# 0x002A/MuCHSALSA

Hardware: AMD Instinct MI355X
Metric: overlap-pairs/s (higher is better)
Workload: dtype int32+f64; 1 GPU; 100k synthetic Nanopore x10 kb, 500k unitig anchors, 10x coverage (BASELINE.json configs[2]); rows=5059558, reads=100000, anchors=499992, edges=981460, edgematches_rank0=25532466, orders_rank0=1029308, parallelism=one job on one GPU, edges_proven_clean_rank0=5372

## Files before the change

### include/msgpu.h

```cpp
#ifndef MSGPU_H
#define MSGPU_H

#include <stddef.h>
#include <stdint.h>

#ifdef __cplusplus
extern "C" {
#endif

#define MSGPU_VERSION 1

#define MSGPU_OK 0
#define MSGPU_E_IO (-1)
#define MSGPU_E_FORMAT (-2)
#define MSGPU_E_NUMBER (-3)
#define MSGPU_E_NOMEM (-4)
#define MSGPU_E_ARG (-5)
#define MSGPU_E_HIP (-6)
#define MSGPU_E_STATE (-7)
#define MSGPU_E_IDS (-8)
#define MSGPU_E_NODEVICE (-9)
#define MSGPU_E_LAYOUT (-10)
#define MSGPU_E_TIMEOUT (-11)

// ... 147 lines not shown


int msgpu_load_rows(msgpu_ctx *ctx, const msgpu_row *rows, size_t n_rows);
int msgpu_load_rows_packed(msgpu_ctx *ctx, const msgpu_packed_rows *packed);
int msgpu_load_rows_device(msgpu_ctx *ctx, const void *d_rows, size_t n_rows);


int msgpu_calculate_edges(msgpu_ctx *ctx);


int msgpu_chaining_and_overlaps(msgpu_ctx *ctx);


int msgpu_get_counts(msgpu_ctx *ctx, msgpu_counts *out);
int msgpu_get_timings(msgpu_ctx *ctx, msgpu_timings *out);
int msgpu_set_stage_events(msgpu_ctx *ctx, int on);

int msgpu_copy_tables(msgpu_ctx *ctx, msgpu_edge *edges, msgpu_edgematch *ems, msgpu_order *orders, uint32_t *ids);
int msgpu_copy_tables_device(msgpu_ctx *ctx, void *d_edges, void *d_ems, void *d_orders, void *d_ids);
int msgpu_copy_reads(msgpu_ctx *ctx, int32_t *read_len, uint32_t *read_first_line);

int msgpu_merge_gathered(msgpu_ctx *ctx, const void *d_gathered, uint32_t world, const uint64_t *counts,
                         uint64_t slab_bytes, uint64_t off_edges, uint64_t off_orders, uint64_t off_ids, void *d_edges,
                         void *d_orders, void *d_ids);

int msgpu_merge_gathered_ex(msgpu_ctx *ctx, const void *d_gathered, uint32_t world, const uint64_t *counts,
                            uint64_t slab_bytes, uint64_t off_edges, uint64_t off_orders, uint64_t off_ids,
                            const uint32_t *id_base, void *d_edges, void *d_orders, void *d_ids, void *hip_stream);

uint64_t msgpu_wire_edges_bytes(uint64_t n_edges);
// ... 336 lines not shown
```

### muchsalsa_amd/_lib.py

```python
import ctypes as C
import os

import numpy as np

_HERE = os.path.dirname(os.path.abspath(__file__))
LIB_PATH = os.environ.get("MSGPU_LIB") or os.path.join(_HERE, "libmsgpu.so")

ROW_DTYPE = np.dtype([("anchor_id", "<u4"), ("read_id", "<u4"), ("read_len", "<i4"), ("i_lo", "<i4"),
                      ("i_hi", "<i4"), ("n_lo", "<i4"), ("n_hi", "<i4"), ("score", "<u4"), ("line", "<u4"),
                      ("flags", "<u4")])
EDGE_DTYPE = np.dtype([("v1", "<u4"), ("v2", "<u4"), ("em_off", "<u8"), ("order_off", "<u8"), ("em_cnt", "<u4"),
                       ("order_cnt", "<u2"), ("shadow", "u1"), ("pad", "u1")])
EM_DTYPE = np.dtype([("ov_lo", "<i4"), ("ov_hi", "<i4"), ("score", "<f8"), ("anchor_id", "<u4"), ("line", "<u4"),
                     ("flags", "<u4"), ("edge_idx", "<u4")])
ORDER_DTYPE = np.dtype([("edge_idx", "<u4"), ("flags", "<u4"), ("left_offset", "<f8"), ("right_offset", "<f8"),
                        ("score", "<u8"), ("ids_off", "<u8"), ("ids_cnt", "<u4"), ("start", "<u4"), ("end", "<u4"),
                        ("base", "<u4"), ("pad", "<u4", (2,))])
COPY_DTYPE = np.dtype([("src_off", "<u8"), ("dst_off", "<u8"), ("len", "<u4"), ("flags", "<u4")])
assert (ROW_DTYPE.itemsize, EDGE_DTYPE.itemsize, EM_DTYPE.itemsize, ORDER_DTYPE.itemsize) == (40, 32, 32, 64)
assert COPY_DTYPE.itemsize == 24
COPY_ILLUMINA, COPY_REVCOMP = 1, 2
PATH_READ_DTYPE = np.dtype([("read_id", "<u4"), ("direction", "<u4"), ("nanopore_length", "<u8")])
PATH_ORDER_DTYPE = np.dtype([("score", "<u8"), ("base_read", "<u4"), ("ids_off", "<u4"), ("ids_cnt", "<u4"),
                             ("pad", "<u4")])
# ... 111 lines not shown
    ("msgpu_parse_paf", C.c_int, [C.c_char_p, C.POINTER(Params), C.POINTER(C.c_void_p)]),
    ("msgpu_paf_free", None, [C.c_void_p]),
    ("msgpu_paf_rows", C.c_void_p, [C.c_void_p, C.POINTER(C.c_size_t)]),
    ("msgpu_paf_line_count", C.c_size_t, [C.c_void_p]),
    ("msgpu_paf_read_count", C.c_uint32, [C.c_void_p]),
    ("msgpu_paf_anchor_count", C.c_uint32, [C.c_void_p]),
    ("msgpu_paf_read_name", C.c_char_p, [C.c_void_p, C.c_uint32]),
    ("msgpu_paf_anchor_name", C.c_char_p, [C.c_void_p, C.c_uint32]),
    ("msgpu_paf_register_sequences", C.c_int, [C.c_void_p, C.c_int, C.c_void_p, C.c_void_p, C.POINTER(C.c_uint32)]),
    ("msgpu_load_rows", C.c_int, [C.c_void_p, C.c_void_p, C.c_size_t]),
    ("msgpu_load_rows_device", C.c_int, [C.c_void_p, C.c_void_p, C.c_size_t]),
    ("msgpu_calculate_edges", C.c_int, [C.c_void_p]),
    ("msgpu_chaining_and_overlaps", C.c_int, [C.c_void_p]),
    ("msgpu_get_counts", C.c_int, [C.c_void_p, C.POINTER(Counts)]),
    ("msgpu_get_timings", C.c_int, [C.c_void_p, C.POINTER(Timings)]),
    ("msgpu_set_stage_events", C.c_int, [C.c_void_p, C.c_int]),
    ("msgpu_copy_tables", C.c_int, [C.c_void_p, C.c_void_p, C.c_void_p, C.c_void_p, C.c_void_p]),
    ("msgpu_copy_tables_device", C.c_int, [C.c_void_p, C.c_void_p, C.c_void_p, C.c_void_p, C.c_void_p]),
    ("msgpu_copy_reads", C.c_int, [C.c_void_p, C.c_void_p, C.c_void_p]),
    ("msgpu_merge_gathered", C.c_int, [C.c_void_p, C.c_void_p, C.c_uint32, C.c_void_p, C.c_uint64, C.c_uint64,
                                       C.c_uint64, C.c_uint64, C.c_void_p, C.c_void_p, C.c_void_p]),
    ("msgpu_merge_gathered_ex", C.c_int, [C.c_void_p, C.c_void_p, C.c_uint32, C.c_void_p, C.c_uint64, C.c_uint64,
                                          C.c_uint64, C.c_uint64, C.c_void_p, C.c_void_p, C.c_void_p, C.c_void_p,
                                          C.c_void_p]),
    ("msgpu_wire_edges_bytes", C.c_uint64, [C.c_uint64]),
    ("msgpu_wire_orders_bytes", C.c_uint64, [C.c_uint64]),
    ("msgpu_wire_ids_bytes", C.c_uint64, [C.c_uint64, C.c_uint32]),
    ("msgpu_pack_wire", C.c_int, [C.c_void_p, C.c_void_p, C.c_void_p, C.c_void_p, C.c_uint32]),
    ("msgpu_merge_wire", C.c_int, [C.c_void_p, C.c_void_p, C.c_uint32, C.c_void_p, C.c_uint64, C.c_uint64, C.c_uint64,
                                   C.c_uint64, C.c_uint32, C.c_void_p, C.c_void_p, C.c_void_p, C.c_void_p, C.c_void_p]),
# ... 167 lines not shown
```

### muchsalsa_amd/csrc/msgpu_api.hip

```cpp
#include <hip/hip_runtime.h>

#include <chrono>
#include <cmath>
#include <cstdarg>
#include <cstdio>
#include <cstdlib>
#include <cstring>
#include <condition_variable>
#include <deque>
#include <mutex>
#include <new>
#include <thread>
#include <vector>
#include <algorithm>
#include <sys/mman.h>
#include <unistd.h>

#include "asm_internal.h"
#include "host_pool.h"
#include "msgpu.h"
#include "msgpu_internal.h"

using namespace msgpu;

// ... 207 lines not shown
  uint32_t V = 0, A = 0;
  const msgpu_row *d_rows = nullptr;

  uint64_t n_edges = 0, n_ems = 0, n_orders = 0, n_ids = 0, n_visit = 0, total_bound = 0;
  uint32_t n_list[4] = {0, 0, 0, 0};

  DevBuf rows_in, rows_pk, cnt_read, read_off, cursor, bkt_key, bkt_dead, by_read, read_cnt, alive_rank,
      anchor_cnt, anchor_off, anchor_first, anchor_off_gen, bkt2_idx, bkt2_line, by_anchor, read_len, read_first, scalars,
      scan_tmp, vis16, spos2, visits, bin_cursor, bin_start;
  DevBuf bound, cand_off, cand_j, cand_t, scr_v2, scr_start, n_cand, n_edge, lists, edges, edge_cand;
  DevBuf big_key, big_t, big_r2s, big_pfx, pair_tab, chain_chunks, big_off, cand_sums, bucket_visits;
  hipStream_t side_stream = nullptr, side_stream2 = nullptr;
  hipEvent_t  ev_side[2]  = {nullptr, nullptr}, ev_side2 = nullptr;
  uint64_t    n_big_edges = 0, n_big_ems = 0;
  bool   fast_path = true;
  bool   sub_wave  = true;
  bool   use_fork  = true;
  bool   use_prologue = true;
  bool   chain_serial = false;
  uint32_t n_cls[4] = {0, 0, 0, 0};
  uint64_t n_edges_fast = 0;
  DevBuf ems, order_scr, ids_scr, edge_norders, edge_nids, orders, ids, big_list, cls_list, big_elems,
      big_paths;
  DevBuf g_deg, g_off, g_adj, g_cand, g_sane, g_out;
  DevBuf sel_idx, sel_cnt, sel_off, sel_ems;

  DevBuf      alt_edges, alt_ems, alt_orders, alt_ids;
  hipStream_t copy_stream = nullptr;
  hipEvent_t  ev_done[2] = {nullptr, nullptr}, ev_copied[2] = {nullptr, nullptr}, ev_wall[2] = {nullptr, nullptr};
  struct HostBuf {
    void  *p   = nullptr;
    size_t cap = 0;
  } h_edges, h_ems, h_orders, h_ids, h_read_len, h_read_first, h_sel_off, h_sel_ems, h_wire[2];
  hipEvent_t ev_part[2][3] = {{nullptr, nullptr, nullptr}, {nullptr, nullptr, nullptr}};
  std::mutex              gate_m;
  std::condition_variable gate_cv;
// ... 470 lines not shown
    return MSGPU_E_HIP;
  }
  c->stream = c->own_stream;
  if (hipHostMalloc(reinterpret_cast<void **>(&c->h_scalars), (SC_COUNT + 1) * sizeof(uint64_t),
                    hipHostMallocMapped | hipHostMallocCoherent) != hipSuccess) {
    c->h_scalars = nullptr;
    msgpu_destroy(c);
    return MSGPU_E_NOMEM;
  }
  memset(c->h_scalars, 0, (SC_COUNT + 1) * sizeof(uint64_t));
  if (hipHostGetDevicePointer(reinterpret_cast<void **>(&c->h_scalars_dev), c->h_scalars, 0) != hipSuccess) c->h_scalars_dev = nullptr;
  c->readback_mapped = c->h_scalars_dev && !getenv("MSGPU_SYNC_READBACK");
  {
    const char *nf = getenv("MSGPU_NO_FASTPATH");
    c->fast_path   = !(nf && nf[0] == '1');
    const char *ns = getenv("MSGPU_NO_SUBWAVE");
    c->sub_wave    = !(ns && ns[0] == '1');
    const char *nw = getenv("MSGPU_NO_WIRE_COPY");
    c->wire_copy   = !(nw && nw[0] == '1');
    const char *nbin = getenv("MSGPU_NO_BIN");
    c->use_bin       = !(nbin && nbin[0] == '1');
    c->use_prologue = !getenv("MSGPU_NO_PROLOGUE");
    c->use_fork     = !getenv("MSGPU_NO_FORK");
    c->chain_serial = getenv("MSGPU_CHAIN_SERIAL") != nullptr;
  }
  for (auto &ev : c->ev)
    if (hipEventCreate(&ev) != hipSuccess) {
      msgpu_destroy(c);
      return MSGPU_E_HIP;
    }
// ... 392 lines not shown
  a.n_edges      = E;
  a.cand_j       = c->cand_j.as<uint32_t>();
  a.cand_t       = c->cand_t.as<uint32_t>();
  a.read_off     = c->read_off.as<uint32_t>();
  a.read_cnt     = c->read_cnt.as<uint32_t>();
  a.read_len     = c->read_len.as<int32_t>();
  a.by_read      = c->by_read.as<IRow>();
  a.by_anchor    = c->by_anchor.as<IRow>();
  a.ems          = c->ems.as<msgpu_edgematch>();
  a.order_scr    = c->order_scr.as<msgpu_order>();
  a.ids_scr      = c->ids_scr.as<uint32_t>();
  a.edge_norders = c->edge_norders.as<uint32_t>();
  a.edge_nids    = c->edge_nids.as<uint32_t>();
  a.err          = scalar<uint32_t>(c, SC_ERR);
  if (!c->pair_tab.p) {
    ENSURE(c, pair_tab, 4 * PAIR_TAB_STRIDE * sizeof(uint32_t) + PAIR_TAB_STRIDE * sizeof(uint2) + 3 * PAIR_TAB_STRIDE * 8);
    launch_fill_pair_tab(st, c->pair_tab.as<uint32_t>());
  }
  a.pair_tab     = c->pair_tab.as<uint32_t>();
  a.pair_tab64   = c->pair_tab.as<uint32_t>() + 4 * PAIR_TAB_STRIDE;
  a.pair_tab_sub = c->pair_tab.as<uint32_t>() + 4 * PAIR_TAB_STRIDE + 2 * PAIR_TAB_STRIDE;
  if (!c->chain_zeroed)
    HIPCHK(c, hipMemsetAsync(c->chain_chunks.p, 0, chunk_words(E) * 8, st));
  c->chain_zeroed = false;
  a.chunk_sums   = c->chain_chunks.as<unsigned long long>();
  a.fast_path    = c->fast_path ? 1 : 0;
  a.fast_margin  = static_cast<long long>(std::min<uint64_t>(c->p.wiggle_room, uint64_t(1) << 40)) - 3;
  a.wiggle       = static_cast<double>(c->p.wiggle_room);
  a.ratio_pct    = c->p.ratio_pct;
  a.alt_frac     = c->p.alt_frac;
  a.out_edge_base = static_cast<uint32_t>(c->base_edges);

  const uint32_t n_big = static_cast<uint32_t>(c->n_big_edges);
  if (n_big) {
    ENSURE(c, big_elems, (c->n_big_ems ? c->n_big_ems : 1) * big_elem_bytes());
    ENSURE(c, big_paths, (c->n_big_ems ? c->n_big_ems : 1) * 2 * big_path_bytes());
  }
  if (n_big) HIPCHK(c, hipEventRecord(c->ev_side[0], st));
  auto launch_big = [&]() -> int {
    if (!n_big) return MSGPU_OK;
    HIPCHK(c, hipStreamWaitEvent(c->side_stream, c->ev_side[0], 0));
// ... 90 lines not shown
int msgpu_get_counts(msgpu_ctx *c, msgpu_counts *out) {
  if (!c || !out) return MSGPU_E_ARG;
  memset(out, 0, sizeof(*out));
  out->n_rows_in       = c->n_rows;
  out->n_rows_alive    = c->n_alive;
  out->n_reads         = c->V;
  out->n_anchors       = c->A;
  out->n_edges         = c->state >= ST_EDGES ? c->n_edges : 0;
  out->n_ems           = c->state >= ST_EDGES ? c->n_ems : 0;
  out->n_orders        = c->state >= ST_CHAINED ? c->n_orders : 0;
  out->n_ids           = c->state >= ST_CHAINED ? c->n_ids : 0;
  out->n_pairs_scanned = c->state >= ST_EDGES ? c->n_visit : 0;
  out->n_edges_fastpath = c->state >= ST_CHAINED ? c->n_edges_fast : 0;
  out->n_lost_publications = c->lost_publications;
  out->index_path          = c->index_path;
  return MSGPU_OK;
}

int msgpu_get_timings(msgpu_ctx *c, msgpu_timings *out) {
  if (!c || !out) return MSGPU_E_ARG;
  memset(out, 0, sizeof(*out));
  HIPCHK(c, hipStreamSynchronize(c->stream));
  if (c->have_index_t) HIPCHK(c, hipEventElapsedTime(&out->index_ms, c->ev[0], c->ev[1]));
  if (c->have_cand_t) HIPCHK(c, hipEventElapsedTime(&out->candidates_ms, c->ev[2], c->ev[3]));
  if (c->have_chain_t) {
    if (c->have_stage_t) {
      HIPCHK(c, hipEventElapsedTime(&out->chain_ms, c->ev[4], c->ev[7]));
      HIPCHK(c, hipEventElapsedTime(&out->compact_ms, c->ev[7], c->ev[8]));
    }
    double   sum = 0;
// ... 721 lines not shown
```

### muchsalsa_amd/csrc/msgpu_internal.h

```cpp
#ifndef MSGPU_INTERNAL_H
#define MSGPU_INTERNAL_H

#include <hip/hip_runtime.h>
#include <stdint.h>

#include "msgpu.h"

namespace msgpu {

struct IRow {
  int32_t  n_lo, n_hi, i_lo, i_hi;
  uint32_t score, line, other, pf;
};
static_assert(sizeof(IRow) == 32, "IRow must be 32 bytes");
constexpr uint32_t PF_POS_MASK = 0x3fffffffu;
constexpr uint32_t PF_DIR      = 1u << 30;
constexpr uint32_t PF_PRIM     = 1u << 31;

enum { SC_MAXIDS = 0 , SC_ERR = 1, SC_TOTAL_A = 2, SC_TOTAL_B = 3, SC_TOTAL_C = 4, SC_NLISTS = 5 ,
       SC_NBIG = 7, SC_NALIVE = 8, SC_IXFLAGS = 9, SC_BIGSTATS = 10 , SC_BIGCUR = 12 ,
       SC_CLS = 14 ,
       SC_HEADS = 16 , SC_DONE = 17 ,
       SC_OWN = 18 , SC_COUNT = 19 };
static_assert(SC_COUNT <= 64, "one wavefront publishes the whole scalar block (publish_to_host)");
// ... 210 lines not shown
void launch_rank_anchor(hipStream_t st, const uint32_t *anchor_off, uint64_t n_rows, const uint32_t *d_n_alive,
                        const uint32_t *bkt_idx, const uint32_t *bkt_line, const msgpu_row *rows,
                        const uint32_t *alive_rank, IRow *by_anchor, const uint32_t *flags, const uint32_t *read_off,
                        IRow *by_read, uint4 *vis);
void launch_bound(hipStream_t st, const uint32_t *read_off, const uint32_t *read_cnt, const uint4 *vis, uint32_t V,
                  uint32_t shard, uint32_t nshards, uint32_t lo, uint32_t hi, uint32_t *bound);
void launch_classify_reads(hipStream_t st, const uint32_t *read_off, const uint32_t *read_cnt, const uint32_t *bound,
                           const uint64_t *cand_off, uint32_t V, uint32_t shard, uint32_t nshards, uint32_t lo,
                           uint32_t hi, CandDesc *l0, CandDesc *l1, CandDesc *l2, uint32_t *l3, uint32_t *n_lists, const CandZero &z,
                           unsigned long long *own_total = nullptr);
void launch_candidates(hipStream_t st, const CandArgs &a, int cls, const CandDesc *list, uint32_t n_list);
void launch_candidates_big(hipStream_t st, const CandArgs &a, const uint32_t *list, uint32_t n_list, uint64_t *big_key,
                           uint32_t *big_t, uint32_t *big_r2s, uint32_t *big_pfx);
void launch_emit_edges(hipStream_t st, const EmitArgs &a, bool reduce);
constexpr uint32_t PAIR_TAB_STRIDE = 2016 + 128;
void launch_fill_pair_tab(hipStream_t st, uint32_t *tab);
void launch_chain(hipStream_t st, const ChainArgs &a, const uint32_t *list, uint32_t n_list);
void launch_chain_sub(hipStream_t st, const ChainArgs &a, int width, const uint32_t *list, uint32_t n_list);
struct ChainSubLists {
  const uint32_t *list32, *list16, *list8;
  uint32_t        n32, n16, n8, nb32, nb16;
};
void launch_chain_sub_all(hipStream_t st, const ChainArgs &a, const uint32_t *l32, uint32_t n32, const uint32_t *l16, uint32_t n16,
                          const uint32_t *l8, uint32_t n8);
size_t big_elem_bytes();
size_t big_path_bytes();
void launch_chain_big(hipStream_t st, const ChainArgs &a, const uint32_t *big_list, const uint64_t *big_off,
                      uint32_t n_big, void *elems, void *paths);
void launch_merge_gathered(hipStream_t st, const MergeArgs &a);
void launch_degree(hipStream_t st, const msgpu_edge *edges, uint64_t n_edges, uint32_t *deg);
// ... 18 lines not shown
```

### muchsalsa_amd/csrc/msgpu_kernels.hip

```cpp
#include <hip/hip_runtime.h>
#include <stdint.h>
#include <stdlib.h>

#include <type_traits>
#include <utility>

#include "msgpu.h"
#include "msgpu_internal.h"
#include "msgpu_device.h"

namespace msgpu {


constexpr int SCAN_ITEMS = 8;
uint32_t      scan_blocks(uint64_t n);

template <class T> __global__ __launch_bounds__(256) void k_scan_reduce(const uint32_t *in, uint64_t n, T *block_sums) {
  __shared__ T s[4];
  uint64_t     base = static_cast<uint64_t>(blockIdx.x) * 256 * SCAN_ITEMS;
  T            sum  = 0;
  for (int i = 0; i < SCAN_ITEMS; ++i) {
    uint64_t idx = base + static_cast<uint64_t>(i) * 256 + threadIdx.x;
    if (idx < n) sum += in[idx];
  }
// ... 1284 lines not shown
        a.big_off[i]  = atomicAdd(&a.big_cursor[1], static_cast<unsigned long long>(ed.em_cnt));
      } else if (ed.em_cnt) {
        a.list[atomicAdd(&s_pos[ed.em_cnt - 1], 1u)] = static_cast<uint32_t>(eb + e);
      }
    }
  }
}
void launch_emit_edges(hipStream_t st, const EmitArgs &a, bool reduce) {
  if (reduce && a.n_chunks)
    hipLaunchKernelGGL(k_cand_reduce, dim3(a.n_chunks), dim3(1024), 0, st, a.n_edge, a.n_cand, a.cand_off, a.edge_scr_start, a.V,
                       const_cast<unsigned long long *>(a.chunk_sums), const_cast<uint32_t *>(a.hist));
  hipLaunchKernelGGL(k_emit_edges, dim3(a.n_chunks ? a.n_chunks : 1), dim3(1024), 0, st, a);
}


__device__ __forceinline__ void chunk_add(unsigned long long *chunk_sums, uint64_t e, bool clean, uint32_t n_orders, uint32_t n_ids) {
  unsigned long long *c = chunk_sums + 2 * (e / COMPACT_CHUNK);
  __hip_atomic_fetch_add(c, (clean ? 1ull : 0ull) | (static_cast<unsigned long long>(n_orders) << 32), __ATOMIC_RELAXED, __HIP_MEMORY_SCOPE_AGENT);
  __hip_atomic_fetch_add(c + 1, static_cast<unsigned long long>(n_ids), __ATOMIC_RELAXED, __HIP_MEMORY_SCOPE_AGENT);
}

struct PathRec {
  uint64_t mask;
  uint64_t score;
  uint32_t primary;
  uint32_t pad;
};

struct __attribute__((aligned(16))) ChainElem {
  double clo1, chi1;
  double clo2, chi2;
  int    rlo1, rhi1, rlo2, rhi2;
};

// ... 208 lines not shown
      x.rlo2 = m2.n_lo;
      x.rhi2 = m2.n_hi;
      x.clo2 = static_cast<double>(m2.n_lo) + ncl2;
      x.chi2 = static_cast<double>(m2.n_hi) - ncr2;
      ovr2   = static_cast<double>(len2 - m2.n_hi) + ncr2;
    }
    clo1     = x.clo1;
    clo2     = x.clo2;
    el[lane] = x;
  }
  const unsigned long long m_plus = __ballot(act && em_dir), m_minus = __ballot(act && !em_dir);
  __builtin_amdgcn_fence(__ATOMIC_RELEASE, "wavefront");
  __builtin_amdgcn_wave_barrier();

  bool clean = false;
  if ((m_plus == 0 || m_minus == 0) && n >= 2 && a.fast_path) {
    const bool      plus = m_minus == 0;
    const ChainElem Pv   = el[lane > 0 ? lane - 1 : 0];
    bool            good = true;
    if (act && lane > 0) {
      good = (Pv.clo1 < x.clo1) & (Pv.chi1 < x.chi1) & (Pv.rlo1 < x.rlo1) & (Pv.rhi1 < x.rhi1);
      good &= plus ? ((Pv.clo2 < x.clo2) & (Pv.chi2 < x.chi2) & (Pv.rlo2 < x.rlo2) & (Pv.rhi2 < x.rhi2))
                   : ((Pv.clo2 > x.clo2) & (Pv.chi2 > x.chi2) & (Pv.rlo2 > x.rlo2) & (Pv.rhi2 > x.rhi2));
    }
    const double av = plus ? x.clo1 - x.clo2 : x.clo1 + x.chi2;
    const double bv = plus ? x.chi1 - x.chi2 : x.chi1 + x.clo2;
    good &= (av > -1.0e9) & (av < 1.0e9) & (bv > -1.0e9) & (bv < 1.0e9) & (em_score > 1.0e-6);
    if (__ballot(act && !good) == 0) {
      int a_hi = act ? static_cast<int>(ceil(av)) : -2147483647 - 1;
      int a_lo = act ? static_cast<int>(floor(av)) : 2147483647;
      int b_hi = act ? static_cast<int>(ceil(bv)) : -2147483647 - 1;
      int b_lo = act ? static_cast<int>(floor(bv)) : 2147483647;
#pragma unroll
      for (int d = 32; d > 0; d >>= 1) {
        a_hi = max(a_hi, __shfl_xor(a_hi, d));
        a_lo = min(a_lo, __shfl_xor(a_lo, d));
        b_hi = max(b_hi, __shfl_xor(b_hi, d));
        b_lo = min(b_lo, __shfl_xor(b_lo, d));
      }
      clean = static_cast<long long>(a_hi) - b_lo <= a.fast_margin && static_cast<long long>(b_hi) - a_lo <= a.fast_margin;
    }
  }

  const int P = __builtin_amdgcn_readfirstlane(clean ? 0 : static_cast<int>(n * (n - 1) / 2));
  static_assert(sizeof(ChainElem) == 48, "the pair table holds byte offsets of 48-byte elements");
  const __amdgpu_buffer_rsrc_t tab_rsrc =
      __builtin_amdgcn_make_buffer_rsrc(const_cast<uint32_t *>(a.pair_tab64), 0, PAIR_TAB_STRIDE * 8, 0x00020000);
  const uint32_t tab_lane = static_cast<uint32_t>(lane) * 8u;
  typedef uint32_t pair_t __attribute__((ext_vector_type(2)));
  auto           load_pairs = [&](int p0) __attribute__((always_inline)) -> pair_t {
    return __builtin_amdgcn_raw_buffer_load_b64(tab_rsrc, tab_lane, p0 * 8, 0);
  };
  double wiggle = a.wiggle;
  asm volatile("" : "+v"(wiggle));
  bool wf_lane = true;
  if (act) {
    const int prev_rlo1 = el[lane > 0 ? lane - 1 : 0].rlo1;
    wf_lane = (x.clo1 <= x.chi1) & (x.clo2 <= x.chi2) & (x.rlo1 <= x.rhi1) & (lane == 0 || prev_rlo1 <= x.rlo1);
  }
  const bool wf = __ballot(!wf_lane) == 0;
  uint32_t cm_addr = CHAIN_LDS_CM;
  asm volatile("" : "+v"(cm_addr));
  auto sweep_step = [&](const int step, const pair_t kl, auto wft, auto dirt, auto s2t) __attribute__((always_inline)) {
    typedef decltype(wft)  WFT;
    typedef decltype(dirt) DIRT;
    typedef decltype(s2t)  S2T;
    constexpr int          DIR = DIRT::value;
    unsigned long long     bits = 0;
    {
      typedef unsigned long long M;
      M valid = ~0ull, KD = 0;
      if (DIR == 2) {
        const int  k = static_cast<int>((kl.x - CHAIN_LDS_EL) / 48u), l = static_cast<int>((kl.y - CHAIN_LDS_EL) / 48u);
        const bool kd = (m_plus >> k) & 1ull, ld = (m_plus >> l) & 1ull;
        valid = __ballot(kd == ld);
// ... 57 lines not shown
  };
  typedef std::integral_constant<int, 0> I0;
  typedef std::integral_constant<int, 1> I1;
  typedef std::integral_constant<int, 2> I2;
  if (wf) {
    if (m_minus == 0) sweep(std::true_type{}, I0{}, I0{});
    else if (m_plus == 0) sweep(std::true_type{}, I1{}, I0{});
    else sweep(std::true_type{}, I2{}, I0{});
  } else {
    if (m_minus == 0) sweep(std::false_type{}, I0{}, I0{});
    else if (m_plus == 0) sweep(std::false_type{}, I1{}, I0{});
    else sweep(std::false_type{}, I2{}, I0{});
  }
  __builtin_amdgcn_fence(__ATOMIC_RELEASE, "wavefront");
  __builtin_amdgcn_wave_barrier();
  uint64_t mycm = 0;
  if (clean) {
    mycm = act ? (1ull << lane) - 1ull : 0ull;
  } else if (act && lane > 0 && P != 0) {
    const int      pr = lane * (lane - 1) / 2, w = pr >> 6, b = pr & 63;
    const uint64_t lo = cm[w] >> b, hi = (cm[w + 1] << 1) << (63 - b);
    mycm              = (lo | hi) & ((1ull << lane) - 1ull);
  }

  double   pop = em_score;
  uint64_t pm  = 1ull << lane;
  {
    uint32_t pred = static_cast<uint32_t>(lane);
    uint32_t rev = __builtin_bitreverse32(static_cast<uint32_t>(mycm));
    const int n1 = static_cast<int>(n) - 1, nlo = n1 < 32 ? n1 : 32;
    auto dp_step = [&](int k) __attribute__((always_inline)) {
      const double       k_pop = rl_f64(pop, k);
      const double       cand  = k_pop + em_score;
      unsigned long long comp, saved;
      asm volatile("v_add_co_u32 %0, %1, %0, %0" : "+v"(rev), "=s"(comp));
      const unsigned long long upd = comp & __ballot(cand > pop);
      asm volatile("s_and_saveexec_b64 %[sv], %[m]\n\t"
                   "v_mov_b64 %[pop], %[cand]\n\t"
                   "v_mov_b32 %[pred], %[k]\n\t"
                   "s_mov_b64 exec, %[sv]"
                   : [pop] "+v"(pop), [pred] "+v"(pred), [sv] "=&s"(saved)
                   : [m] "s"(upd), [cand] "v"(cand), [k] "s"(k)
                   : "scc");
    };
    for (int k = 0; k < nlo; ++k) dp_step(k);
    rev = __builtin_bitreverse32(static_cast<uint32_t>(mycm >> 32));
    for (int k = 32; k < n1; ++k) dp_step(k);
    uint32_t ptr = pred;
    for (uint32_t span = 1; span < n; span <<= 1) {
      const uint32_t lo = __shfl(static_cast<uint32_t>(pm), static_cast<int>(ptr));
      const uint32_t hi = __shfl(static_cast<uint32_t>(pm >> 32), static_cast<int>(ptr));
      const uint32_t p2 = __shfl(ptr, static_cast<int>(ptr));
      pm |= (static_cast<uint64_t>(hi) << 32) | lo;
      ptr = p2;
    }
  }

  PathRec  *pmn = reinterpret_cast<PathRec *>(s_chain_lds + CHAIN_LDS_EL), *ppl = pmn + 64;
  const int n_m = paths_of_direction(m_minus, false, lane, pop, pm, em_prim, j1, q2, n1, n2, a.alt_frac, pmn);
  const int n_p = paths_of_direction(m_plus, true, lane, pop, pm, em_prim, j1, q2, n1, n2, a.alt_frac, ppl);
  __builtin_amdgcn_fence(__ATOMIC_RELEASE, "wavefront");
  __builtin_amdgcn_wave_barrier();

  bool     k_m = false, k_p = false;
  uint32_t prim_m = 0, prim_p = 0, len_m = 0, len_p = 0;
  if (lane < n_m) {
    prim_m = pmn[lane].primary;
    len_m  = static_cast<uint32_t>(__popcll(pmn[lane].mask));
    k_m    = true;
  }
  if (lane < n_p) {
// ... 79 lines not shown
        o.start        = (fl & MSGPU_ORD_START_V1) ? v1 : v2;
        o.end          = (fl & MSGPU_ORD_START_V1) ? v2 : v1;
        o.base         = v1;
        o.pad[0]       = 0;
        o.pad[1]       = 0;
        a.order_scr[ed.em_off + n_orders] = o;
      }
      ++n_orders;
      n_ids += cnt;
    }
  }
  if (lane == 0) {
    a.edge_norders[e] = n_orders;
    a.edge_nids[e]    = n_ids;
    a.edges[e].shadow = shadow ? 1 : 0;
    chunk_add(a.chunk_sums, e, clean, n_orders, n_ids);
  }
}


struct __attribute__((aligned(16))) SubPath {
  uint32_t mask, primary;
  uint64_t score;
};

__device__ __forceinline__ double shfl_f64(double v, int src) {
  const long long b  = __double_as_longlong(v);
  const uint32_t  lo = __shfl(static_cast<uint32_t>(b), src), hi = __shfl(static_cast<uint32_t>(b >> 32), src);
  return __longlong_as_double(static_cast<long long>((static_cast<unsigned long long>(hi) << 32) | lo));
}

// ... 187 lines not shown
    clo2     = x.clo2;
    el[lane] = x;
  }
  {
    double *kp = s_keep[wave][lane];
    kp[0] = clo1, kp[1] = clo2, kp[2] = ovr1, kp[3] = ovr2;
    s_anchor[wave][lane] = anchor;
  }
  const uint32_t m_plus  = group_bits<W>(__ballot(act && em_dir), gbase);
  const uint32_t m_minus = group_bits<W>(__ballot(act && !em_dir), gbase);
  __builtin_amdgcn_fence(__ATOMIC_RELEASE, "wavefront");
  __builtin_amdgcn_wave_barrier();

  bool clean = false;
  {
    const bool      try_clean = (m_plus == 0 || m_minus == 0) && n >= 2 && a.fast_path;
    const bool      plus      = m_minus == 0;
    const ChainElem Pv        = el[sl > 0 ? lane - 1 : lane];
    bool            good      = true;
    if (act && sl > 0) {
      good = (Pv.clo1 < x.clo1) & (Pv.chi1 < x.chi1) & (Pv.rlo1 < x.rlo1) & (Pv.rhi1 < x.rhi1);
      good &= plus ? ((Pv.clo2 < x.clo2) & (Pv.chi2 < x.chi2) & (Pv.rlo2 < x.rlo2) & (Pv.rhi2 < x.rhi2))
                   : ((Pv.clo2 > x.clo2) & (Pv.chi2 > x.chi2) & (Pv.rlo2 > x.rlo2) & (Pv.rhi2 > x.rhi2));
    }
    const double av = plus ? x.clo1 - x.clo2 : x.clo1 + x.chi2;
    const double bv = plus ? x.chi1 - x.chi2 : x.chi1 + x.clo2;
    good &= (av > -1.0e9) & (av < 1.0e9) & (bv > -1.0e9) & (bv < 1.0e9) & (em_score > 1.0e-6);
    const bool maybe = try_clean && group_bits<W>(__ballot(act && !good), gbase) == 0;
    if (__ballot(maybe)) {
      int a_hi = act ? static_cast<int>(ceil(av)) : -2147483647 - 1;
      int a_lo = act ? static_cast<int>(floor(av)) : 2147483647;
// ... 725 lines not shown
    a.edges[e].shadow = shadow ? 1 : 0;
    chunk_add(a.chunk_sums, e, false, n_orders, n_ids);
  }
}

__device__ __forceinline__ void tab64_entry(uint32_t *tab, int p, int k, int l, int run) {
  (void)run;
  tab[4 * PAIR_TAB_STRIDE + 2 * p]     = static_cast<uint32_t>(k * 48);
  tab[4 * PAIR_TAB_STRIDE + 2 * p + 1] = static_cast<uint32_t>(l * 48);
}
__device__ __forceinline__ void tabsub_entry(uint32_t *tab, int t, int p, int k, int l, int run) {
  uint32_t *e = tab + 4 * PAIR_TAB_STRIDE + 2 * PAIR_TAB_STRIDE + (static_cast<size_t>(t - 1) * PAIR_TAB_STRIDE + p) * 2;
  e[0]        = static_cast<uint32_t>(k * 48) | (static_cast<uint32_t>(l * 48) << 16);
  e[1]        = static_cast<uint32_t>(k) | (static_cast<uint32_t>(run) << 8) | (static_cast<uint32_t>(l * 4) << 16);
}
__global__ __launch_bounds__(256) void k_fill_pair_tab(uint32_t *tab) {
  const int i = blockIdx.x * 256 + threadIdx.x;
  if (i >= 4 * static_cast<int>(PAIR_TAB_STRIDE)) return;
  const int t = i / static_cast<int>(PAIR_TAB_STRIDE), p = i % static_cast<int>(PAIR_TAB_STRIDE), W = 64 >> t;
  if (p >= 2016) {
    tab[i] = 1u << 8;
    if (t == 0) tab64_entry(tab, p, 0, 1, 0);
    else tabsub_entry(tab, t, p, 0, 1, 0);
    return;
  }
  int l = static_cast<int>((1.0f + __fsqrt_rn(1.0f + 8.0f * static_cast<float>(p))) * 0.5f);
  if (l * (l - 1) / 2 > p) --l;
  if ((l + 1) * l / 2 <= p) ++l;
  const int k = p - l * (l - 1) / 2, lane = p % W;
  const int run = (k == 0 || lane == 0) ? min(l - k, W - lane) : 0;
  tab[i] = static_cast<uint32_t>(k | (l << 8) | (run << 16)) | (static_cast<uint32_t>(64 - run - k) << 24);
  if (t == 0) tab64_entry(tab, p, k, l, run);
  else tabsub_entry(tab, t, p, k, l, run);
}

__global__ __launch_bounds__(1024) __attribute__((amdgpu_waves_per_eu(8, 8))) void k_compact(CompactArgs a) {
  __shared__ unsigned long long s_red[16][5], s_tot[5], s_em[COMPACT_CHUNK];
  __shared__ uint32_t           s_ob[COMPACT_CHUNK], s_ib[COMPACT_CHUNK], s_no[COMPACT_CHUNK], s_w[2][16];
  static_assert(COMPACT_CHUNK == 1024, "an edge per thread");
  const int      lane = threadIdx.x & 63, wave = threadIdx.x >> 6;
  const uint32_t chunk = blockIdx.x;
  const uint64_t my_e  = static_cast<uint64_t>(chunk) * COMPACT_CHUNK + threadIdx.x;
  const uint32_t my_no = my_e < a.n_edges ? a.edge_norders[my_e] : 0u, my_ni = my_e < a.n_edges ? a.edge_nids[my_e] : 0u;
  const uint64_t my_em = my_e < a.n_edges ? a.edges[my_e].em_off : 0ull;
  unsigned long long t[5] = {0, 0, 0, 0, 0};
  for (uint32_t c = threadIdx.x; c < a.n_chunks; c += 1024) {
    const unsigned long long w0 = a.chunk_sums[2 * c], w1 = a.chunk_sums[2 * c + 1];
    const unsigned long long no = w0 >> 32, nf = w0 & 0xffffffffull;
    if (c < chunk) {
      t[0] += no;
      t[1] += w1;
    }
    t[2] += no;
    t[3] += w1;
    t[4] += nf;
  }
#pragma unroll
  for (int k = 0; k < 5; ++k) {
    for (int d = 32; d > 0; d >>= 1) t[k] += __shfl_xor(t[k], d);
    if (lane == 0) s_red[wave][k] = t[k];
  }
  __syncthreads();
  if (wave == 0) {
// ... 440 lines not shown
```

### muchsalsa_amd/overlap.py

```python
import ctypes as C
import os

import numpy as np

from . import _lib
from ._lib import EDGE_DTYPE, EM_DTYPE, ORDER_DTYPE, ROW_DTYPE, Counts, HostTables, Params, Timings


class MsgpuError(RuntimeError):
    def __init__(self, code, detail=""):
        msg = _lib.lib().msgpu_strerror(code).decode()
        super().__init__("%s (%d)%s" % (msg, code, (": " + detail) if detail else ""))
        self.code = code


def default_params():
    p = Params()
    _lib.lib().msgpu_default_params(C.byref(p))
    return p


class Paf:

    def __init__(self, rows, n_lines, read_names, anchor_names, handle=None, n_reads=None, n_anchors=None):
# ... 166 lines not shown

    def calculate_edges(self):
        self._check(self._L.msgpu_calculate_edges(self._h))

    def chaining_and_overlaps(self):
        self._check(self._L.msgpu_chaining_and_overlaps(self._h))

    def synchronize(self):
        self._check(self._L.msgpu_synchronize(self._h))

    def counts(self):
        c = Counts()
        self._check(self._L.msgpu_get_counts(self._h, C.byref(c)))
        return c

    def set_stage_events(self, on):
        self._check(self._L.msgpu_set_stage_events(self._h, 1 if on else 0))

    def timings(self):
        t = Timings()
        self._check(self._L.msgpu_get_timings(self._h, C.byref(t)))
        return t

    def tables(self):
        c = self.counts()
        edges = np.zeros(c.n_edges, dtype=EDGE_DTYPE)
        ems = np.zeros(c.n_ems, dtype=EM_DTYPE)
        orders = np.zeros(c.n_orders, dtype=ORDER_DTYPE)
        ids = np.zeros(c.n_ids, dtype="<u4")
        self._check(self._L.msgpu_copy_tables(self._h, edges.ctypes.data, ems.ctypes.data, orders.ctypes.data,
# ... 173 lines not shown
```

Before: 421.9 million overlap-pairs/s.

## Add banded pair sweep to chaining kernel with exact fallback check

For non-clean edges with more than band+1 elements, the 64-lane chaining kernel now evaluates only predecessor pairs within a fixed band (default 12) instead of all n(n-1)/2 pairs, using a new band table appended to the pair table. After the DP it verifies, via a prefix max of scores, that no out-of-band predecessor could improve any lane's score. If any could, it reruns the full triangular sweep and counts a fallback. This cuts the quadratic pair work for long chains, at the cost of an extra verification scan and a possible double sweep. It also adds debug counters packed into the chunk sums.

After: 434.3 million overlap-pairs/s, median of 6. 2.9% higher.

```diff
diff --git a/include/msgpu.h b/include/msgpu.h
--- a/include/msgpu.h
+++ b/include/msgpu.h
@@ -185,6 +185,8 @@
 
 int msgpu_get_counts(msgpu_ctx *ctx, msgpu_counts *out);
 int msgpu_get_timings(msgpu_ctx *ctx, msgpu_timings *out);
+int msgpu_get_chain_band_counts(msgpu_ctx *ctx, uint64_t *n_banded, uint64_t *n_fallback);
+int msgpu_chain_band_width(void);
 int msgpu_set_stage_events(msgpu_ctx *ctx, int on);
 
 int msgpu_copy_tables(msgpu_ctx *ctx, msgpu_edge *edges, msgpu_edgematch *ems, msgpu_order *orders, uint32_t *ids);
diff --git a/muchsalsa_amd/_lib.py b/muchsalsa_amd/_lib.py
--- a/muchsalsa_amd/_lib.py
+++ b/muchsalsa_amd/_lib.py
@@ -149,6 +149,8 @@
     ("msgpu_chaining_and_overlaps", C.c_int, [C.c_void_p]),
     ("msgpu_get_counts", C.c_int, [C.c_void_p, C.POINTER(Counts)]),
     ("msgpu_get_timings", C.c_int, [C.c_void_p, C.POINTER(Timings)]),
+    ("msgpu_get_chain_band_counts", C.c_int, [C.c_void_p, C.POINTER(C.c_uint64), C.POINTER(C.c_uint64)]),
+    ("msgpu_chain_band_width", C.c_int, []),
     ("msgpu_set_stage_events", C.c_int, [C.c_void_p, C.c_int]),
     ("msgpu_copy_tables", C.c_int, [C.c_void_p, C.c_void_p, C.c_void_p, C.c_void_p, C.c_void_p]),
     ("msgpu_copy_tables_device", C.c_int, [C.c_void_p, C.c_void_p, C.c_void_p, C.c_void_p, C.c_void_p]),
diff --git a/muchsalsa_amd/csrc/msgpu_api.hip b/muchsalsa_amd/csrc/msgpu_api.hip
--- a/muchsalsa_amd/csrc/msgpu_api.hip
+++ b/muchsalsa_amd/csrc/msgpu_api.hip
@@ -245,12 +245,14 @@
   hipEvent_t  ev_side[2]  = {nullptr, nullptr}, ev_side2 = nullptr;
   uint64_t    n_big_edges = 0, n_big_ems = 0;
   bool   fast_path = true;
+  bool   chain_band = true;
   bool   sub_wave  = true;
   bool   use_fork  = true;
   bool   use_prologue = true;
   bool   chain_serial = false;
   uint32_t n_cls[4] = {0, 0, 0, 0};
   uint64_t n_edges_fast = 0;
+  uint64_t chain_E = 0;
   DevBuf ems, order_scr, ids_scr, edge_norders, edge_nids, orders, ids, big_list, cls_list, big_elems,
       big_paths;
   DevBuf g_deg, g_off, g_adj, g_cand, g_sane, g_out;
@@ -751,6 +753,8 @@
   {
     const char *nf = getenv("MSGPU_NO_FASTPATH");
     c->fast_path   = !(nf && nf[0] == '1');
+    const char *nb = getenv("MSGPU_NO_BAND");
+    c->chain_band  = c->fast_path && !(nb && nb[0] == '1');
     const char *ns = getenv("MSGPU_NO_SUBWAVE");
     c->sub_wave    = !(ns && ns[0] == '1');
     const char *nw = getenv("MSGPU_NO_WIRE_COPY");
@@ -1173,7 +1177,7 @@
   a.edge_nids    = c->edge_nids.as<uint32_t>();
   a.err          = scalar<uint32_t>(c, SC_ERR);
   if (!c->pair_tab.p) {
-    ENSURE(c, pair_tab, 4 * PAIR_TAB_STRIDE * sizeof(uint32_t) + PAIR_TAB_STRIDE * sizeof(uint2) + 3 * PAIR_TAB_STRIDE * 8);
+    ENSURE(c, pair_tab, PAIR_TAB_WORDS * sizeof(uint32_t));
     launch_fill_pair_tab(st, c->pair_tab.as<uint32_t>());
   }
   a.pair_tab     = c->pair_tab.as<uint32_t>();
@@ -1183,7 +1187,8 @@
     HIPCHK(c, hipMemsetAsync(c->chain_chunks.p, 0, chunk_words(E) * 8, st));
   c->chain_zeroed = false;
   a.chunk_sums   = c->chain_chunks.as<unsigned long long>();
-  a.fast_path    = c->fast_path ? 1 : 0;
+  a.fast_path    = (c->fast_path ? CHAIN_FAST_SHORTCUT : 0) | (c->chain_band ? CHAIN_FAST_BAND : 0);
+  c->chain_E     = E;
   a.fast_margin  = static_cast<long long>(std::min<uint64_t>(c->p.wiggle_room, uint64_t(1) << 40)) - 3;
   a.wiggle       = static_cast<double>(c->p.wiggle_room);
   a.ratio_pct    = c->p.ratio_pct;
@@ -1304,6 +1309,23 @@
   out->n_edges_fastpath = c->state >= ST_CHAINED ? c->n_edges_fast : 0;
   out->n_lost_publications = c->lost_publications;
   out->index_path          = c->index_path;
+  return MSGPU_OK;
+}
+
+int msgpu_chain_band_width(void) { return MSGPU_CHAIN_BAND; }
+
+int msgpu_get_chain_band_counts(msgpu_ctx *c, uint64_t *n_banded, uint64_t *n_fallback) {
+  if (!c || !n_banded || !n_fallback) return MSGPU_E_ARG;
+  *n_banded = *n_fallback = 0;
+  if (c->state < ST_CHAINED || !c->chain_chunks.p) return MSGPU_OK;
+  HIPCHK(c, hipSetDevice(c->device));
+  const size_t n_chunks = static_cast<size_t>((c->chain_E + COMPACT_CHUNK - 1) / COMPACT_CHUNK);
+  const size_t fb_word  = 2 * static_cast<size_t>(c->chain_E / COMPACT_CHUNK + 1);
+  std::vector<unsigned long long> w(fb_word + 1);
+  HIPCHK(c, hipStreamSynchronize(c->stream));
+  HIPCHK(c, hipMemcpy(w.data(), c->chain_chunks.p, w.size() * 8, hipMemcpyDeviceToHost));
+  for (size_t k = 0; k < n_chunks; ++k) *n_banded += (w[2 * k] >> 16) & 0xffffull;
+  *n_fallback = w[fb_word];
   return MSGPU_OK;
 }
 
diff --git a/muchsalsa_amd/csrc/msgpu_internal.h b/muchsalsa_amd/csrc/msgpu_internal.h
--- a/muchsalsa_amd/csrc/msgpu_internal.h
+++ b/muchsalsa_amd/csrc/msgpu_internal.h
@@ -248,6 +248,15 @@
                            uint32_t *big_t, uint32_t *big_r2s, uint32_t *big_pfx);
 void launch_emit_edges(hipStream_t st, const EmitArgs &a, bool reduce);
 constexpr uint32_t PAIR_TAB_STRIDE = 2016 + 128;
+#ifndef MSGPU_CHAIN_BAND
+#define MSGPU_CHAIN_BAND 12
+#endif
+static_assert(MSGPU_CHAIN_BAND >= 1 && MSGPU_CHAIN_BAND <= 62, "band width");
+constexpr int chain_band_pairs(int n) { return MSGPU_CHAIN_BAND * (MSGPU_CHAIN_BAND + 1) / 2 + (n - 1 - MSGPU_CHAIN_BAND) * MSGPU_CHAIN_BAND; }
+static_assert(chain_band_pairs(64) <= 2016, "the band table fits the stride of the others");
+constexpr uint32_t PAIR_TAB_BAND64_OFF = 4 * PAIR_TAB_STRIDE + 2 * PAIR_TAB_STRIDE + 3 * 2 * PAIR_TAB_STRIDE;
+constexpr uint32_t PAIR_TAB_WORDS      = PAIR_TAB_BAND64_OFF + 2 * PAIR_TAB_STRIDE;
+constexpr int CHAIN_FAST_SHORTCUT = 1, CHAIN_FAST_BAND = 2;
 void launch_fill_pair_tab(hipStream_t st, uint32_t *tab);
 void launch_chain(hipStream_t st, const ChainArgs &a, const uint32_t *list, uint32_t n_list);
 void launch_chain_sub(hipStream_t st, const ChainArgs &a, int width, const uint32_t *list, uint32_t n_list);
diff --git a/muchsalsa_amd/csrc/msgpu_kernels.hip b/muchsalsa_amd/csrc/msgpu_kernels.hip
--- a/muchsalsa_amd/csrc/msgpu_kernels.hip
+++ b/muchsalsa_amd/csrc/msgpu_kernels.hip
@@ -1322,10 +1322,14 @@
 }
 
 
-__device__ __forceinline__ void chunk_add(unsigned long long *chunk_sums, uint64_t e, bool clean, uint32_t n_orders, uint32_t n_ids) {
+__device__ __forceinline__ void chunk_add(unsigned long long *chunk_sums, uint64_t e, bool clean, uint32_t n_orders, uint32_t n_ids, bool banded = false) {
+  static_assert(COMPACT_CHUNK < (1u << 16), "two 16-bit edge counts in the low half of a chunk sum");
   unsigned long long *c = chunk_sums + 2 * (e / COMPACT_CHUNK);
-  __hip_atomic_fetch_add(c, (clean ? 1ull : 0ull) | (static_cast<unsigned long long>(n_orders) << 32), __ATOMIC_RELAXED, __HIP_MEMORY_SCOPE_AGENT);
+  __hip_atomic_fetch_add(c, (clean ? 1ull : 0ull) | (banded ? 1ull << 16 : 0ull) | (static_cast<unsigned long long>(n_orders) << 32), __ATOMIC_RELAXED, __HIP_MEMORY_SCOPE_AGENT);
   __hip_atomic_fetch_add(c + 1, static_cast<unsigned long long>(n_ids), __ATOMIC_RELAXED, __HIP_MEMORY_SCOPE_AGENT);
+}
+__device__ __forceinline__ void band_fallback_add(unsigned long long *chunk_sums, uint64_t n_edges) {
+  __hip_atomic_fetch_add(chunk_sums + 2 * (n_edges / COMPACT_CHUNK + 1), 1ull, __ATOMIC_RELAXED, __HIP_MEMORY_SCOPE_AGENT);
 }
 
 struct PathRec {
@@ -1564,7 +1568,7 @@
   __builtin_amdgcn_wave_barrier();
 
   bool clean = false;
-  if ((m_plus == 0 || m_minus == 0) && n >= 2 && a.fast_path) {
+  if ((m_plus == 0 || m_minus == 0) && n >= 2 && (a.fast_path & CHAIN_FAST_SHORTCUT)) {
     const bool      plus = m_minus == 0;
     const ChainElem Pv   = el[lane > 0 ? lane - 1 : 0];
     bool            good = true;
@@ -1592,10 +1596,21 @@
     }
   }
 
-  const int P = __builtin_amdgcn_readfirstlane(clean ? 0 : static_cast<int>(n * (n - 1) / 2));
+  bool wf_lane = true;
+  if (act) {
+    const int prev_rlo1 = el[lane > 0 ? lane - 1 : 0].rlo1;
+    wf_lane = (x.clo1 <= x.chi1) & (x.clo2 <= x.chi2) & (x.rlo1 <= x.rhi1) & (lane == 0 || prev_rlo1 <= x.rlo1);
+  }
+  const bool wf = __ballot(!wf_lane) == 0;
+  bool     band = !clean && (a.fast_path & CHAIN_FAST_BAND) && n > MSGPU_CHAIN_BAND + 1;
+  const bool banded = band;
+  double   pop;
+  uint64_t pm;
+  for (;;) {
+  const int P = __builtin_amdgcn_readfirstlane(clean ? 0 : band ? chain_band_pairs(static_cast<int>(n)) : static_cast<int>(n * (n - 1) / 2));
   static_assert(sizeof(ChainElem) == 48, "the pair table holds byte offsets of 48-byte elements");
   const __amdgpu_buffer_rsrc_t tab_rsrc =
-      __builtin_amdgcn_make_buffer_rsrc(const_cast<uint32_t *>(a.pair_tab64), 0, PAIR_TAB_STRIDE * 8, 0x00020000);
+      __builtin_amdgcn_make_buffer_rsrc(const_cast<uint32_t *>(a.pair_tab64) + (band ? PAIR_TAB_BAND64_OFF - 4 * PAIR_TAB_STRIDE : 0u), 0, PAIR_TAB_STRIDE * 8, 0x00020000);
   const uint32_t tab_lane = static_cast<uint32_t>(lane) * 8u;
   typedef uint32_t pair_t __attribute__((ext_vector_type(2)));
   auto           load_pairs = [&](int p0) __attribute__((always_inline)) -> pair_t {
@@ -1603,12 +1618,6 @@
   };
   double wiggle = a.wiggle;
   asm volatile("" : "+v"(wiggle));
-  bool wf_lane = true;
-  if (act) {
-    const int prev_rlo1 = el[lane > 0 ? lane - 1 : 0].rlo1;
-    wf_lane = (x.clo1 <= x.chi1) & (x.clo2 <= x.chi2) & (x.rlo1 <= x.rhi1) & (lane == 0 || prev_rlo1 <= x.rlo1);
-  }
-  const bool wf = __ballot(!wf_lane) == 0;
   uint32_t cm_addr = CHAIN_LDS_CM;
   asm volatile("" : "+v"(cm_addr));
   auto sweep_step = [&](const int step, const pair_t kl, auto wft, auto dirt, auto s2t) __attribute__((always_inline)) {
@@ -1696,19 +1705,24 @@
   }
   __builtin_amdgcn_fence(__ATOMIC_RELEASE, "wavefront");
   __builtin_amdgcn_wave_barrier();
+  int ln = lane;
+  asm volatile("" : "+v"(ln));
   uint64_t mycm = 0;
   if (clean) {
-    mycm = act ? (1ull << lane) - 1ull : 0ull;
-  } else if (act && lane > 0 && P != 0) {
-    const int      pr = lane * (lane - 1) / 2, w = pr >> 6, b = pr & 63;
+    mycm = act ? (1ull << ln) - 1ull : 0ull;
+  } else if (act && ln > 0 && P != 0) {
+    constexpr int  B  = MSGPU_CHAIN_BAND;
+    const bool     tri = !band || ln <= B;
+    const int      pr = tri ? ln * (ln - 1) / 2 : B * (B - 1) / 2 + (ln - B) * B, w = pr >> 6, b = pr & 63;
+    const int      wd = tri ? ln : B;
     const uint64_t lo = cm[w] >> b, hi = (cm[w + 1] << 1) << (63 - b);
-    mycm              = (lo | hi) & ((1ull << lane) - 1ull);
-  }
-
-  double   pop = em_score;
-  uint64_t pm  = 1ull << lane;
+    mycm              = ((lo | hi) & ((1ull << wd) - 1ull)) << (ln - wd);
+  }
+
+  pop = em_score;
+  pm  = 1ull << ln;
   {
-    uint32_t pred = static_cast<uint32_t>(lane);
+    uint32_t pred = static_cast<uint32_t>(ln);
     uint32_t rev = __builtin_bitreverse32(static_cast<uint32_t>(mycm));
     const int n1 = static_cast<int>(n) - 1, nlo = n1 < 32 ? n1 : 32;
     auto dp_step = [&](int k) __attribute__((always_inline)) {
@@ -1737,6 +1751,23 @@
       ptr = p2;
     }
   }
+  if (!band) break;
+  {
+    double pmax = pop;
+#pragma unroll
+    for (int d = 1; d < 64; d <<= 1) {
+      const double up = __shfl_up(pmax, d);
+      if (ln >= d) pmax = __builtin_fmax(pmax, up);
+    }
+    const double out = __shfl(pmax, ln > MSGPU_CHAIN_BAND ? ln - MSGPU_CHAIN_BAND - 1 : 0);
+    const bool   rej = ln > MSGPU_CHAIN_BAND && ln < static_cast<int>(n) && !(out + em_score < pop);
+    if (__ballot(rej) == 0) break;
+  }
+  band = false;
+  if (lane == 0) band_fallback_add(a.chunk_sums, a.n_edges);
+  __builtin_amdgcn_fence(__ATOMIC_RELEASE, "wavefront");
+  __builtin_amdgcn_wave_barrier();
+  }
 
   PathRec  *pmn = reinterpret_cast<PathRec *>(s_chain_lds + CHAIN_LDS_EL), *ppl = pmn + 64;
   const int n_m = paths_of_direction(m_minus, false, lane, pop, pm, em_prim, j1, q2, n1, n2, a.alt_frac, pmn);
@@ -1846,7 +1877,7 @@
     a.edge_norders[e] = n_orders;
     a.edge_nids[e]    = n_ids;
     a.edges[e].shadow = shadow ? 1 : 0;
-    chunk_add(a.chunk_sums, e, clean, n_orders, n_ids);
+    chunk_add(a.chunk_sums, e, clean, n_orders, n_ids, banded);
   }
 }
 
@@ -2064,7 +2095,7 @@
 
   bool clean = false;
   {
-    const bool      try_clean = (m_plus == 0 || m_minus == 0) && n >= 2 && a.fast_path;
+    const bool      try_clean = (m_plus == 0 || m_minus == 0) && n >= 2 && (a.fast_path & CHAIN_FAST_SHORTCUT);
     const bool      plus      = m_minus == 0;
     const ChainElem Pv        = el[sl > 0 ? lane - 1 : lane];
     bool            good      = true;
@@ -2820,10 +2851,31 @@
   e[0]        = static_cast<uint32_t>(k * 48) | (static_cast<uint32_t>(l * 48) << 16);
   e[1]        = static_cast<uint32_t>(k) | (static_cast<uint32_t>(run) << 8) | (static_cast<uint32_t>(l * 4) << 16);
 }
+__device__ __forceinline__ void band64_entry(uint32_t *tab, int p) {
+  constexpr int B = MSGPU_CHAIN_BAND, TRI = B * (B + 1) / 2;
+  int k = 0, l = 1;
+  if (p < TRI) {
+    l = static_cast<int>((1.0f + __fsqrt_rn(1.0f + 8.0f * static_cast<float>(p))) * 0.5f);
+    if (l * (l - 1) / 2 > p) --l;
+    if ((l + 1) * l / 2 <= p) ++l;
+    k = p - l * (l - 1) / 2;
+  } else {
+    const int q = p - TRI;
+    l = B + 1 + q / B;
+    k = l - B + q % B;
+    if (l >= 64) {
+      k = 0;
+      l = 1;
+    }
+  }
+  tab[PAIR_TAB_BAND64_OFF + 2 * p]     = static_cast<uint32_t>(k * 48);
+  tab[PAIR_TAB_BAND64_OFF + 2 * p + 1] = static_cast<uint32_t>(l * 48);
+}
 __global__ __launch_bounds__(256) void k_fill_pair_tab(uint32_t *tab) {
   const int i = blockIdx.x * 256 + threadIdx.x;
   if (i >= 4 * static_cast<int>(PAIR_TAB_STRIDE)) return;
   const int t = i / static_cast<int>(PAIR_TAB_STRIDE), p = i % static_cast<int>(PAIR_TAB_STRIDE), W = 64 >> t;
+  if (t == 0) band64_entry(tab, p);
   if (p >= 2016) {
     tab[i] = 1u << 8;
     if (t == 0) tab64_entry(tab, p, 0, 1, 0);
@@ -2852,7 +2904,7 @@
   unsigned long long t[5] = {0, 0, 0, 0, 0};
   for (uint32_t c = threadIdx.x; c < a.n_chunks; c += 1024) {
     const unsigned long long w0 = a.chunk_sums[2 * c], w1 = a.chunk_sums[2 * c + 1];
-    const unsigned long long no = w0 >> 32, nf = w0 & 0xffffffffull;
+    const unsigned long long no = w0 >> 32, nf = w0 & 0xffffull;
     if (c < chunk) {
       t[0] += no;
       t[1] += w1;
diff --git a/muchsalsa_amd/overlap.py b/muchsalsa_amd/overlap.py
--- a/muchsalsa_amd/overlap.py
+++ b/muchsalsa_amd/overlap.py
@@ -204,6 +204,14 @@
         self._check(self._L.msgpu_get_counts(self._h, C.byref(c)))
         return c
 
+    def chain_band_counts(self):
+        nb, nf = C.c_uint64(0), C.c_uint64(0)
+        self._check(self._L.msgpu_get_chain_band_counts(self._h, C.byref(nb), C.byref(nf)))
+        return int(nb.value), int(nf.value)
+
+    def chain_band_width(self):
+        return int(self._L.msgpu_chain_band_width())
+
     def set_stage_events(self, on):
         self._check(self._L.msgpu_set_stage_events(self._h, 1 if on else 0))
 
```
